# pymc-devs/nutpie

Hardware: AMD Instinct MI355X
Metric: leapfrog steps/sec (all chains) (higher is better)
Workload: dtype f64

## Files before the change

### nutpie_amd/csrc/kernels.hip

```cpp
#include <hip/hip_runtime.h>

#include "../../include/nphip_spec.h"
#include "engine_types.h"
#include "kernel_families.h"

#if defined(__HIP_DEVICE_COMPILE__)
#define NPHIP_GLOBAL __attribute__((address_space(1)))
#define NPHIP_LDS __attribute__((address_space(3)))
#define NPHIP_CONST __attribute__((address_space(4)))
#else
#define NPHIP_GLOBAL
#define NPHIP_LDS
#define NPHIP_CONST
#endif

#ifdef NPHIP_JIT_DENSITY
#define NPHIP_JIT 1
#else
#define NPHIP_JIT 0
#endif

namespace nphip {


// ... 392 lines not shown
                                       LdsDouble edge_ = nullptr)
        : A(a), c(ctl), red(r), par(par_), ring(ring_), edge(edge_), chain(ch), gchain((uint32_t)(a.chain_offset + ch)) {
        lane = threadIdx.x & 63;
        wave = (W == 1) ? 0 : __builtin_amdgcn_readfirstlane((int)(threadIdx.x >> 6));
        D = a.dim; ld = a.ld; nch = ld / NPHIP_CHUNK;
        qp = a.qpool + (size_t)ch * a.nqpool * 2 * ld;
        pp = a.pslots + (size_t)ch * a.npslots * ((NV == -1 || LR) ? (size_t)a.pvec : (size_t)2) * ld;
        sig2 = a.sig2 + (size_t)ch * ld;
        est = a.est + (size_t)ch * 8 * ld;
        T = a.s.num_tune + a.s.num_draws;
        if (DENS) {
            extern __shared__ __attribute__((aligned(16))) double s_dyn_dens[];
            const int slot = (W == 1) ? __builtin_amdgcn_readfirstlane((int)(threadIdx.x >> 6)) : 0;
            dens_lds = (LdsDouble)s_dyn_dens + (size_t)slot * a.dens_lds_doubles;
            dens_shared = (LdsDouble)s_dyn_dens + (size_t)(W == 1 ? 4 : 1) * a.dens_lds_doubles;
            dens_rows = dens_shared + a.dens_shared_doubles + (size_t)slot * 2 * ld;
        }
    }

    __device__ __forceinline__ void qe_st(int64_t i, double2 v) const { st2_dense(A.qeval + (size_t)chain * D, i, D, v); }
    __device__ __forceinline__ double2 ge_ld(int64_t i) const {
        const double* row = A.geval + (size_t)chain * D;
        if (DG && !(A.dg_variant & 128)) {
            double2 v;
            v.x = (i < D) ? __hip_atomic_load(row + i, __ATOMIC_RELAXED, __HIP_MEMORY_SCOPE_AGENT) : 0.0;
            v.y = (i + 1 < D) ? __hip_atomic_load(row + i + 1, __ATOMIC_RELAXED, __HIP_MEMORY_SCOPE_AGENT) : 0.0;
            return v;
        }
        return ld2_dense(row, i, D);
    }
    __device__ __forceinline__ double* Q(int64_t b) const { return qp + (size_t)b * 2 * ld; }
    __device__ __forceinline__ double* G(int64_t b) const { return qp + (size_t)b * 2 * ld + ld; }
    __device__ __forceinline__ size_t pvec() const { return LRK ? (size_t)A.pvec : (size_t)2; }
    __device__ __forceinline__ double* P(int64_t s) const { return pp + (size_t)s * pvec() * ld; }
    __device__ __forceinline__ double* R(int64_t s) const { return pp + (size_t)s * pvec() * ld + ld; }
    __device__ __forceinline__ double* VEL(int64_t s) const { return pp + (size_t)s * pvec() * ld + 2 * ld; }
    static constexpr bool LRK = NV == -1 || LR;
    __device__ __forceinline__ bool lr_job() const { return LRK && A.lr_on != 0; }
    __device__ __forceinline__ const float* LRV(int j) const { return A.lr_V + ((size_t)chain * kLrMax + j) * ld; }
    __device__ __forceinline__ double* EST(int64_t e, int k) const { return est + (size_t)(e * 4 + k) * ld; }
    __device__ __forceinline__ bool leader() const { return lane == 0 && wave == 0; }
    template <int N>
    __device__ __forceinline__ void rsum(double (&v)[N]) {
        static_assert(N <= 16, "a reduction area holds 16 values per wave");
        reduceN<W, N, false, !LEAN>(v, red + (W > 1 ? rflip * 16 * W : 0));
        rflip ^= 1;
    }
    __device__ __forceinline__ void rsum2(double& a, double& b) {
        double v[2] = {a, b};
        rsum(v);
        a = v[0]; b = v[1];
    }
    __device__ __forceinline__ double2 sg2(int64_t i) const {
        if (sig_lds) { const double2 v = *(const NPHIP_LDS double2*)(sig_lds + i); return v; }
        return ld2(sig2, i);
    }
    __device__ __forceinline__ double sg1(int64_t i) const { return sig_lds ? sig_lds[i] : ld1(sig2, i); }

#define NPHIP_FOR_CHUNKS(i) for (int64_t cc_ = wave, i = cc_ * NPHIP_CHUNK + 2 * lane; cc_ < nch; cc_ += W, i = cc_ * NPHIP_CHUNK + 2 * lane)
    template <int U, class LoadT, class BodyT>
    __device__ __forceinline__ void chunks_pf(LoadT load, BodyT body) const {
        for (int64_t c0 = wave; c0 < nch; c0 += (int64_t)W * U) {
            decltype(load((int64_t)0)) v[U];
#pragma unroll
            for (int u = 0; u < U; ++u) {
                int64_t cc = c0 + (int64_t)u * W;
                cc = cc < nch ? cc : nch - 1;
                v[u] = load(cc * NPHIP_CHUNK + 2 * lane);
            }
#pragma unroll
            for (int u = 0; u < U; ++u) {
                const int64_t cc = c0 + (int64_t)u * W;
                if (cc < nch) body(cc * NPHIP_CHUNK + 2 * lane, v[u]);
            }
        }
    }
    static constexpr bool BATCHED = (W == 1);
#ifdef NPHIP_NO_PFRARE
    static constexpr bool PFRARE = false;
#else
    static constexpr bool PFRARE = FUSED && W == 1 && NV >= 2 && !LEAN;
#endif
    static constexpr bool ENDOUT = FUSED && W == 1 && NV >= 2 && !LEAN;
    template <class LoadT, class BodyT>
    __device__ __forceinline__ void chunks(LoadT load, BodyT body) const {
        if (nch > 2) chunks_pf<4>(load, body);
        else chunks_pf<2>(load, body);
    }
    struct V4 { double2 a, b, c, d; };

    __device__ void da_init(double step) {
        c->da_log_step = nphip_log(step);
        c->da_log_step_adapted = c->da_log_step;
        c->da_hbar = 0.0;
        c->da_mu = A.s.adapt_adam ? 0.0 : nphip_log(10.0 * step);
        c->adam_b1t = 1.0; c->adam_b2t = 1.0;
        c->da_count = 1;
    }
    __device__ void da_advance(double accept) {
        if (A.s.adapt_adam) {
            const double g = accept - A.s.target_accept;
            c->da_hbar = 0.9 * c->da_hbar + (1.0 - 0.9) * g;
            c->da_mu = 0.999 * c->da_mu + (1.0 - 0.999) * (g * g);
            c->adam_b1t = c->adam_b1t * 0.9; c->adam_b2t = c->adam_b2t * 0.999;
            const double mhat = c->da_hbar / (1.0 - c->adam_b1t), vhat = c->da_mu / (1.0 - c->adam_b2t);
            c->da_log_step = c->da_log_step + A.s.adam_lr * mhat / (sqrt(vhat) + 1e-8);
            c->da_log_step_adapted = c->da_log_step;
            c->da_count += 1;
            return;
        }
        const double cnt = (double)c->da_count;
        double w = 1.0 / (cnt + A.s.da_t0);
        c->da_hbar = (1.0 - w) * c->da_hbar + w * (A.s.target_accept - accept);
        c->da_log_step = c->da_mu - c->da_hbar * sqrt(cnt) / A.s.da_gamma;
        double mk = nphip_exp(-A.s.da_k * nphip_log(cnt));
        c->da_log_step_adapted = mk * c->da_log_step + (1.0 - mk) * c->da_log_step_adapted;
        c->da_count += 1;
    }
    __device__ void update_stepsize(int64_t draw, bool best) {
        if (A.s.fixed_step_size) return;
        double step = best ? nphip_exp(c->da_log_step_adapted) : nphip_exp(c->da_log_step);
        if (A.s.jitter > 0.0) {
            nphip_u32x4 r = nphip_philox(A.s.seed, 0u, gchain, (uint32_t)draw, NPHIP_RNG_JITTER);
            double u = nphip_u01(r.v[0], r.v[1]);
            step *= fma(2.0 * A.s.jitter, u, 1.0 - A.s.jitter);
        }
        if (step > A.s.max_step_size) step = A.s.max_step_size;
        c->step_size = step;
    }
    __device__ int64_t alloc_q(bool in_tree) const {
        uint32_t used = 1u << c->cand_q;
        if (in_tree) {
            used |= (1u << c->endq[0]) | (1u << c->endq[1]) | (1u << c->curq);
            for (uint64_t m = (uint64_t)c->nleaf & ((1ull << kMaxDepthCap) - 1); m != 0; m &= m - 1) used |= 1u << c->sub_q[__builtin_ctzll(m)];
        }
        return (int64_t)__builtin_ctz(~used);
    }
    __device__ void finish_chain(int64_t phase, int64_t err) {
        c->phase = phase;
        c->err = err;
        if (leader()) atomicAdd(&A.counters[phase == PH_ERROR ? 1 : 0], 1ull);
    }

    __device__ void gen_init(int64_t attempt) {
        double* q = Q(0);
        NPHIP_FOR_CHUNKS(i) {
            double2 v = {0.0, 0.0};
            if (A.s.init_kind == 2) {
                v = ld2_dense(A.init_points + (size_t)chain * D, i, D);
            } else if (i < D) {
                nphip_u32x4 r = nphip_philox(A.s.seed, (uint32_t)(i >> 1), gchain, (uint32_t)attempt, NPHIP_RNG_INIT);
                if (A.s.init_kind == 0) {
                    v.x = fma(4.0, nphip_u01(r.v[0], r.v[1]), -2.0);
                    v.y = fma(4.0, nphip_u01(r.v[2], r.v[3]), -2.0);
                } else {
                    nphip_normal_pair(r, &v.x, &v.y);
                }
                if (i + 1 >= D) v.y = 0.0;
            }
            st2(q, i, v);
            if (!FUSED) qe_st(i, v);
        }
        c->eval_buf = 0;
    }

    struct LrAcc { double2 a[kLrMax]; };
// ... 1136 lines not shown
    __device__ __forceinline__ void regs_grad(RegsT& X) {
        double2 z[NVX];
#pragma unroll
        for (int k = 0; k < NVX; ++k) {
            const double2 mu = par_mu(ridx(k));
            z[k].x = X.q[k].x - mu.x;
            z[k].y = X.q[k].y - mu.y;
        }
        publish_edges(z);
#pragma unroll
        for (int k = 0; k < NVX; ++k) {
            double2 a, b01;
            double b2, edge_zl, edge_zr;
            par_ab(ridx(k), a, b01, b2);
            edge_pair(z, k, edge_zl, edge_zr);
            const double zl = wave_shr1(z[k].y, edge_zl), zr = wave_shl1(z[k].x, edge_zr);
            double tx = a.x * z[k].x;
            tx = fma(b01.x, zl, tx);
            tx = fma(b01.y, z[k].y, tx);
            double ty = a.y * z[k].y;
            ty = fma(b01.y, z[k].x, ty);
            ty = fma(b2, zr, ty);
            X.g[k].x = -tx;
            X.g[k].y = -ty;
        }
        if (W > 1) __syncthreads();
    }
    __device__ __forceinline__ void store_state(RegsT& X, bool q_, bool pr) {
        constexpr int nk = NVX;
        if (q_) {
            double* qn = Q(X.reg_q);
#pragma unroll
            for (int k = 0; k < NVX; ++k) if (k < nk) st2(qn, ridx(k), X.q[k]);
            if (REMOTE) {
                double* gn = G(X.reg_q);
#pragma unroll
                for (int k = 0; k < NVX; ++k) if (k < nk) st2(gn, ridx(k), X.g[k]);
            }
            X.dirty_qg = false;
        }
        if (pr) {
            double *pn = P(X.reg_p), *rn = R(X.reg_p);
#pragma unroll
            for (int k = 0; k < NVX; ++k) if (k < nk) { st2(pn, ridx(k), X.p[k]); st2(rn, ridx(k), X.r[k]); }
            if (LR) {
                double* vn = VEL(X.reg_p);
#pragma unroll
                for (int k = 0; k < NVX; ++k) st2(vn, ridx(k), X.v[k]);
            }
            X.dirty_pr = false;
        }
    }
    __device__ __forceinline__ void flush(RegsT& X) {
        if (NV <= 0) return;
        if (X.dirty_qg || X.dirty_pr) { if (LEAN) lean_store(lean_rs(), X, X.dirty_qg, X.dirty_pr); else store_state(X, X.dirty_qg, X.dirty_pr); }
        if (c->phase == PH_TREE) {
            if (LEAN) {
                lean_ring_flush(lean_rs(), X);
            } else {
                const int64_t d = c->depth;
                if (X.ring_leaf0 >= 0) flush_ring_slot(0, first_slot_of(X.ring_leaf0, d));
                if (X.ring_leaf1 >= 0) flush_ring_slot(1, slot_last(__builtin_ctzll((unsigned long long)X.ring_leaf1), A.cap));
            }
        }
    }
    __device__ __forceinline__ void flush_ring_slot(int sl, int64_t slot) {
        constexpr int nk = NVX;
        double2 tp[NVX], tr[NVX];
        ring_read(sl, tp, tr);
        double *pn = P(slot), *rn = R(slot);
#pragma unroll
        for (int k = 0; k < NVX; ++k) if (k < nk) { st2(pn, ridx(k), tp[k]); st2(rn, ridx(k), tr[k]); }
    }

    struct Hot {
        int32_t nleaf, depth, dir, idx_cur;
        int32_t srcq, srcp, newq, newp;
        int32_t n_steps, n_steps0;
        int32_t end_newp;
        uint32_t used_base, sub_used, draw;
        bool check;
        double step, H0, acc, acc_sym, max_ee;
    };
    static __device__ __forceinline__ int32_t end_code(bool diverging, bool maxdepth, bool store_div, bool div_has_end, bool regrad, bool replay) {
        return 1 | (diverging ? 2 : 0) | (maxdepth ? 4 : 0) | (store_div ? 8 : 0) | (div_has_end ? 16 : 0) | (regrad ? 32 : 0) | (replay ? 64 : 0);
    }
    static __device__ __forceinline__ int32_t rfl(int64_t v) { return __builtin_amdgcn_readfirstlane((int)v); }
    static __device__ __forceinline__ double rfl_f64(double v) {
        return __hiloint2double(__builtin_amdgcn_readfirstlane(__double2hiint(v)), __builtin_amdgcn_readfirstlane(__double2loint(v)));
    }
    __device__ __forceinline__ void hot_doubling(Hot& H) const {
        const int db = H.dir > 0 ? 1 : 0;
        H.used_base = (1u << rfl(c->cand_q)) | (1u << rfl(c->endq[0])) | (1u << rfl(c->endq[1]));
        H.end_newp = slot_end(db, (int)(rfl(c->endpar[db]) ^ 1));
        H.check = A.s.check_turning && ((int64_t)H.depth + 1 > A.s.mindepth);
    }
    __device__ __forceinline__ void hot_load(Hot& H) const {
        H.nleaf = rfl(c->nleaf); H.depth = rfl(c->depth); H.dir = rfl(c->dir); H.idx_cur = rfl(c->idx_cur);
        H.srcq = rfl(c->lf_srcq); H.srcp = rfl(c->lf_srcp); H.newq = rfl(c->lf_newq); H.newp = rfl(c->lf_newp);
        H.n_steps = H.n_steps0 = rfl(c->n_steps); H.draw = (uint32_t)rfl(c->draw);
        H.step = rfl_f64(c->step_size); H.H0 = rfl_f64(c->H0); H.acc = rfl_f64(c->acc_sum); H.acc_sym = rfl_f64(c->acc_sym_sum);
        H.max_ee = A.s.max_energy_error;
        hot_doubling(H);
        H.sub_used = 0u;
        for (uint32_t m = (uint32_t)H.nleaf & ((1u << kMaxDepthCap) - 1u); m != 0; m &= m - 1) H.sub_used |= 1u << rfl(c->sub_q[__builtin_ctz(m)]);
    }
    __device__ __forceinline__ void hot_save(Hot& H) {
        c->nleaf = H.nleaf; c->dir = H.dir; c->idx_cur = H.idx_cur;
        c->lf_srcq = H.srcq; c->lf_srcp = H.srcp; c->lf_newq = H.newq; c->lf_newp = H.newp; c->lf_sign = H.dir; c->eval_buf = H.newq;
        c->curq = H.srcq; c->curp = H.srcp;
        c->n_steps = H.n_steps; c->total_steps += (int64_t)(H.n_steps - H.n_steps0);
        H.n_steps0 = H.n_steps;
        c->acc_sum = H.acc; c->acc_sym_sum = H.acc_sym;
    }
    __device__ __forceinline__ void issue_leaf_hot(Hot& H) const {
        const int32_t j = H.nleaf + 1, d = H.depth;
        int32_t newp;
        if (j == (1 << d)) newp = H.end_newp;
        else if (j & 1) newp = (j == 1) ? slot_first(d) : slot_first(__builtin_ctz((unsigned)(j - 1)));
        else newp = slot_last(__builtin_ctz((unsigned)j), A.cap);
        H.newq = (int32_t)__builtin_ctz(~(H.used_base | H.sub_used | (1u << H.srcq)));
        H.newp = newp;
    }
    __device__ __forceinline__ void start_doubling_hot(Hot& H) const {
        nphip_u32x4 r = nphip_philox(A.s.seed, (uint32_t)H.depth, gchain, H.draw, NPHIP_RNG_DIRECTION);
        H.dir = (r.v[0] & 1u) ? 1 : -1;
        const int db = H.dir > 0 ? 1 : 0;
        H.nleaf = 0;
        H.srcq = rfl(c->endq[db]);
        H.srcp = rfl(c->endp[db]);
        H.idx_cur = rfl(H.dir > 0 ? c->idx_right : c->idx_left);
        H.sub_used = 0u;
        hot_doubling(H);
        issue_leaf_hot(H);
    }
    __device__ __forceinline__ double merge_uniform_hot(const Hot& H, int32_t j, int32_t d, int32_t k, nphip_u32x4& blk, int32_t& blk_id) const {
        const int32_t id = k >> 1;
        if (blk_id != id) {
            const uint32_t c3 = (uint32_t)NPHIP_RNG_MERGE | ((uint32_t)d << 8) | ((uint32_t)id << 16);
            blk = nphip_philox(A.s.seed, (uint32_t)j, gchain, H.draw, c3);
            blk_id = id;
        }
        return (k & 1) ? nphip_u01(blk.v[2], blk.v[3]) : nphip_u01(blk.v[0], blk.v[1]);
    }

    __device__ __forceinline__ void merge_level(Hot& H, int32_t j, int32_t d, int32_t k, nphip_u32x4& blk, int32_t& blk_id, double& T_wm, int64_t& T_we,
                                                int32_t& T_q, double& T_U, double& T_E, int32_t& T_idx) {
        double sm; int64_t se;
        const int32_t A_q = rfl(c->sub_q[k]), A_idx = rfl(c->sub_idx[k]);
        const double A_U = c->sub_U[k], A_E = c->sub_E[k];
        H.sub_used &= ~(1u << A_q);
        nphip_w_add(c->sub_wm[k], c->sub_we[k], T_wm, T_we, &sm, &se);
        const bool take = merge_uniform_hot(H, j, d, k, blk, blk_id) * sm < nphip_w_rel(T_wm, T_we, se);
        if (!take) { T_q = A_q; T_U = A_U; T_E = A_E; T_idx = A_idx; }
        T_wm = sm; T_we = se;
    }

    __device__ __forceinline__ bool leaf_reg(RegsT& X, Hot& H, int32_t& end_code_out) {
        constexpr int nk = NVX;
        const int32_t j = H.nleaf + 1, d = H.depth, dir = H.dir;
        const int db = dir > 0 ? 1 : 0;
        const int32_t idx_new = H.idx_cur + dir;
        const int32_t srcq = H.srcq, srcp = H.srcp, newq = H.newq, newp = H.newp;
        const bool check = H.check;
#ifdef NPHIP_PROFILE
        const int64_t tp0 = (int64_t)__builtin_readcyclecounter();
#endif
        if (X.reg_q != srcq) {
            const double* q = Q(srcq);
#pragma unroll
            for (int k = 0; k < NVX; ++k) if (k < nk) X.q[k] = ld2(q, ridx(k));
            if (REMOTE) {
                const double* g = G(srcq);
#pragma unroll
                for (int k = 0; k < NVX; ++k) if (k < nk) X.g[k] = ld2(g, ridx(k));
            } else {
                regs_grad(X);
            }
        }
        if (X.reg_p != srcp) { load_slot(srcp, X.p, X.r); if (LR) load_slot_v(srcp, X.v); }
        if (!X.sig_ok) {
#pragma unroll
            for (int k = 0; k < NVX; ++k) if (k < nk) X.s[k] = ld2(sig2, ridx(k));
            if (LR) {
                const double* sdp = A.lr_std + (size_t)chain * ld;
#pragma unroll
                for (int k = 0; k < NVX; ++k) X.sd[k] = ld2(sdp, ridx(k));
            }
            X.sig_ok = true;
        }
        if (j == 1) { X.ring_leaf0 = -1; X.ring_leaf1 = -1; }
        const bool lrm = LR && lr_job() && rfl(c->host_metric) != 0;
        const int lrk = lrm ? (int)rfl(c->lr_k) : 0;
        NPHIP_PHASE_FENCE();
        const double eps = (double)dir * H.step;
        const double h = 0.5 * eps;
        if (idx_new == -1) {
#pragma unroll
            for (int k = 0; k < NVX; ++k) if (k < nk) { X.r[k].x = -0.0; X.r[k].y = -0.0; }
        }
        double2 z[NVX], pold[NVX], rold[NVX], vold[NVX];
        LrAcc lrS;
        double lrc[kLrMax];
        if (LR && lrm) lr_zero(lrS);
#pragma unroll
        for (int k = 0; k < NVX; ++k) if (k < nk) {
            pold[k] = X.p[k];
            rold[k] = X.r[k];
            if (LR) vold[k] = X.v[k];
            X.p[k].x = fma(h, X.g[k].x, X.p[k].x);
            X.p[k].y = fma(h, X.g[k].y, X.p[k].y);
            if (LR && lrm) {
            } else {
                X.q[k].x = fma(eps, X.s[k].x * X.p[k].x, X.q[k].x);
                X.q[k].y = fma(eps, X.s[k].y * X.p[k].y, X.q[k].y);
            }
            if (!REMOTE && !(LR && lrm)) {
                const double2 mu = par_mu(ridx(k));
                z[k].x = X.q[k].x - mu.x;
                z[k].y = X.q[k].y - mu.y;
            }
        }
        if (LR && lrm) {
            lr_dispatch(lrk, [&](auto kc) {
#pragma unroll
                for (int k = 0; k < NVX; ++k) {
                    double2 u;
                    u.x = X.sd[k].x * X.p[k].x; u.y = X.sd[k].y * X.p[k].y;
                    lr_acc_c<decltype(kc)::value>(lrS, ridx(k), u);
                }
            });
            lr_coef(lrS, lrk, 0, lrc);
            lr_dispatch(lrk, [&](auto kc) {
#pragma unroll
                for (int k = 0; k < NVX; ++k) {
                    double2 u;
                    u.x = X.sd[k].x * X.p[k].x; u.y = X.sd[k].y * X.p[k].y;
                    const double2 w = lr_apply_c<decltype(kc)::value>(ridx(k), u, lrc);
                    X.q[k].x = fma(eps, X.sd[k].x * w.x, X.q[k].x);
                    X.q[k].y = fma(eps, X.sd[k].y * w.y, X.q[k].y);
                }
            });
            if (!REMOTE) {
#pragma unroll
                for (int k = 0; k < NVX; ++k) {
                    const double2 mu = par_mu(ridx(k));
                    z[k].x = X.q[k].x - mu.x;
                    z[k].y = X.q[k].y - mu.y;
                }
            }
        }
        double lp_remote = 0.0;
        int64_t code_remote = 0;
        if (REMOTE) {
            if (DENS) {
#pragma unroll
                for (int k = 0; k < NVX; ++k) if (k < nk) *(NPHIP_LDS double2*)(dens_rows + ridx(k)) = X.q[k];
                remote_eval(lp_remote, code_remote, true);
            } else {
#pragma unroll
                for (int k = 0; k < NVX; ++k) if (k < nk) qe_st(ridx(k), X.q[k]);
                remote_eval(lp_remote, code_remote, false, !DG);
            }
        } else {
            publish_edges(z);
        }
        double2 accK = {0.0, 0.0}, accL = {0.0, 0.0}, accE = {0.0, 0.0}, accS = {0.0, 0.0};
        if (LR && lrm) lr_zero(lrS);
#pragma unroll
        for (int k = 0; k < NVX; ++k) if (k < nk) {
            double2 gg;
            if (DENS) {
                gg = *(const NPHIP_LDS double2*)(dens_rows + ld + ridx(k));
                if (ridx(k) >= D) gg.x = 0.0;
                if (ridx(k) + 1 >= D) gg.y = 0.0;
            } else if (REMOTE) {
                gg = ge_ld(ridx(k));
                if (DG) {
                    const double2 mu = ld2(A.dg_mu, ridx(k));
                    accL.x = fma(X.q[k].x - mu.x, gg.x, accL.x);
                    accL.y = fma(X.q[k].y - mu.y, gg.y, accL.y);
                }
            } else {
                double2 a, b01;
                double b2, edge_zl, edge_zr;
                par_ab(ridx(k), a, b01, b2);
                edge_pair(z, k, edge_zl, edge_zr);
                const double zl = wave_shr1(z[k].y, edge_zl);
                const double zr = wave_shl1(z[k].x, edge_zr);
                double tx = a.x * z[k].x;
                tx = fma(b01.x, zl, tx);
                tx = fma(b01.y, z[k].y, tx);
                double ty = a.y * z[k].y;
                ty = fma(b01.y, z[k].x, ty);
                ty = fma(b2, zr, ty);
                gg.x = -tx;
                gg.y = -ty;
                accL.x = fma(z[k].x, gg.x, accL.x);
                accL.y = fma(z[k].y, gg.y, accL.y);
            }
            X.g[k] = gg;
            X.p[k].x = fma(h, gg.x, X.p[k].x);
            X.p[k].y = fma(h, gg.y, X.p[k].y);
            X.r[k].x = rold[k].x + X.p[k].x;
            X.r[k].y = rold[k].y + X.p[k].y;
            if (LR && lrm) continue;
            const double vx = X.s[k].x * X.p[k].x, vy = X.s[k].y * X.p[k].y;
            accK.x = fma(X.p[k].x, vx, accK.x);
            accK.y = fma(X.p[k].y, vy, accK.y);
            const double tx0 = (X.r[k].x - rold[k].x) + pold[k].x, ty0 = (X.r[k].y - rold[k].y) + pold[k].y;
            accE.x = fma(tx0, vx, accE.x);
            accE.y = fma(ty0, vy, accE.y);
            if (LR) {
                X.v[k].x = vx; X.v[k].y = vy;
                accS.x = fma(tx0, vold[k].x, accS.x);
                accS.y = fma(ty0, vold[k].y, accS.y);
            } else {
                accS.x = fma(tx0, X.s[k].x * pold[k].x, accS.x);
                accS.y = fma(ty0, X.s[k].y * pold[k].y, accS.y);
            }
        }
        if (LR && lrm) {
            lr_dispatch(lrk, [&](auto kc) {
#pragma unroll
                for (int k = 0; k < NVX; ++k) {
                    double2 u;
                    u.x = X.sd[k].x * X.p[k].x; u.y = X.sd[k].y * X.p[k].y;
                    lr_acc_c<decltype(kc)::value>(lrS, ridx(k), u);
                }
            });
            lr_coef(lrS, lrk, 0, lrc);
            lr_dispatch(lrk, [&](auto kc) {
#pragma unroll
                for (int k = 0; k < NVX; ++k) {
                    double2 u;
                    u.x = X.sd[k].x * X.p[k].x; u.y = X.sd[k].y * X.p[k].y;
                    const double2 w = lr_apply_c<decltype(kc)::value>(ridx(k), u, lrc);
                    X.v[k].x = X.sd[k].x * w.x; X.v[k].y = X.sd[k].y * w.y;
                }
            });
#pragma unroll
            for (int k = 0; k < NVX; ++k) {
                accK.x = fma(X.p[k].x, X.v[k].x, accK.x);
                accK.y = fma(X.p[k].y, X.v[k].y, accK.y);
                const double tx0 = (X.r[k].x - rold[k].x) + pold[k].x, ty0 = (X.r[k].y - rold[k].y) + pold[k].y;
                accE.x = fma(tx0, X.v[k].x, accE.x);
                accE.y = fma(ty0, X.v[k].y, accE.y);
                accS.x = fma(tx0, vold[k].x, accS.x);
                accS.y = fma(ty0, vold[k].y, accS.y);
            }
        }
        X.reg_q = newq;
        X.reg_p = newp;
        X.dirty_qg = true;
        X.dirty_pr = true;
        if (!LR && !NORING) {
            if ((j & 3) == 1) { ring_write(0, X.p, X.r); X.ring_leaf0 = j; }
            else if ((j & 3) == 2) { ring_write(1, X.p, X.r); X.ring_leaf1 = j; }
        }
#ifdef NPHIP_PROFILE
        const int64_t tp1 = (int64_t)__builtin_readcyclecounter();
#endif
        NPHIP_PHASE_FENCE();
        double v4[4] = {accK.x + accK.y, accL.x + accL.y, accE.x + accE.y, accS.x + accS.y};
        rsum(v4);
        NPHIP_PHASE_FENCE();
#ifdef NPHIP_PROFILE
        const int64_t tp2 = (int64_t)__builtin_readcyclecounter();
        c->prof[0] += tp1 - tp0; c->prof[6] += tp2 - tp1;
#endif
        const double K = 0.5 * v4[0], lp = (REMOTE && !DG) ? lp_remote : 0.5 * v4[1];
        const bool turn0 = (v4[2] < 0.0) || (v4[3] < 0.0);
        if (REMOTE && code_remote < 0) { X.dirty_qg = X.dirty_pr = false; hot_save(H); finish_chain(PH_ERROR, CE_FATAL_LOGP); return true; }
        H.nleaf += 1;
        H.n_steps += 1;
        const bool ok = isfinite(lp) && (!REMOTE || code_remote == 0);
        const double Unew = -lp, E = K + Unew, dE = E - H.H0;
        const bool diverged = !ok || (dE > H.max_ee) || !isfinite(dE);
        double T_wm = 1.0;
        int64_t T_we = 0;
        nphip_u32x4 mrg_blk = {{0u, 0u, 0u, 0u}};
        int32_t mrg_id = -1;
        {
            if (!diverged) {
                const double x = -dE, xc = x > 1e9 ? 1e9 : (x < -1e9 ? -1e9 : x);
                double kk;
                nphip_exp_parts(xc, &T_wm, &kk);
                T_we = (int64_t)kk;
                const double e = nphip_exp_scale(x, T_wm, kk);
                const double a = e < 1.0 ? e : 1.0;
                H.acc += a;
                H.acc_sym += 2.0 * a / (1.0 + e);
            }
        }
        if (diverged) { X.dirty_qg = X.dirty_pr = false; hot_save(H);
            if (ENDOUT) end_code_out = end_code(true, false, FUSED, ok, !REMOTE, FUSED); else rare_end_draw(A, c, red, chain, true, false, FUSED, ok, !REMOTE, FUSED);
            return true; }
#ifdef NPHIP_PROFILE
        int64_t tq = (int64_t)__builtin_readcyclecounter();
        c->prof[8] += tq - tp2;
#endif

        NPHIP_PHASE_FENCE();
        double T_U = Unew, T_E = E;
        int32_t T_q = newq, T_idx = idx_new;
        H.srcq = newq; H.srcp = newp; H.idx_cur = idx_new;
        double2 obp[NVX], obr[NVX], obv[NVX];
        int32_t k = 0;
        while (k < d && (((j - 1) >> k) & 1)) {
            if (check) {
                bool turn;
                if (k == 0) {
                    turn = turn0;
                } else if (LR) {
                    const int32_t a = j - (2 << k) + 1, al = j - (1 << k);
                    load_slot(first_slot_of(a, d), obp, obr); load_slot_v(first_slot_of(a, d), obv);
                    if (k == 2) { load_slot(first_slot_of(al + 1, d), pold, rold); load_slot_v(first_slot_of(al + 1, d), vold); }
                    turn = sub_a_v(X, obp, obr, obv, pold, rold, vold);
                    if (k >= 2) {
#pragma unroll
                        for (int q_ = 0; q_ < NVX; ++q_) { pold[q_] = obp[q_]; rold[q_] = obr[q_]; vold[q_] = obv[q_]; }
                    }
                    if (!turn) {
                        const int32_t sl_ = slot_last(__builtin_ctz((unsigned)al), A.cap);
                        load_slot(sl_, obp, obr); load_slot_v(sl_, obv);
                        turn = sub_b_v(X, obp, obr, obv);
                    }
                } else {
                    const int32_t a = j - (2 << k) + 1, al = j - (1 << k);
                    if (k == 1 && X.ring_leaf0 == a) ring_read(0, obp, obr);
                    else load_slot(first_slot_of(a, d), obp, obr);
                    if (k == 2) {
                        if (X.ring_leaf0 == al + 1) ring_read(0, pold, rold);
                        else load_slot(first_slot_of(al + 1, d), pold, rold);
                    }
                    turn = sub_a(X, obp, obr, pold, rold);
                    if (k >= 2) {
#pragma unroll
                        for (int q_ = 0; q_ < NVX; ++q_) { pold[q_] = obp[q_]; rold[q_] = obr[q_]; }
                    }
                    if (!turn) {
                        if (k == 1 && X.ring_leaf1 == al) ring_read(1, obp, obr);
                        else load_slot(slot_last(__builtin_ctz((unsigned)al), A.cap), obp, obr);
                        turn = sub_b(X, obp, obr);
                    }
                }
                if (turn) { X.dirty_qg = X.dirty_pr = false; hot_save(H); if (ENDOUT) end_code_out = end_code(false, false, false, false, !REMOTE, false); else rare_end_draw(A, c, red, chain, false, false, false, false, !REMOTE); return true; }
            }
#ifdef NPHIP_PROFILE
            { const int64_t t_ = (int64_t)__builtin_readcyclecounter(); c->prof[k == 0 ? 9 : 10] += t_ - tq; tq = t_; }
#endif
            NPHIP_PHASE_FENCE();
            merge_level(H, j, d, k, mrg_blk, mrg_id, T_wm, T_we, T_q, T_U, T_E, T_idx);
            NPHIP_PHASE_FENCE();
#ifdef NPHIP_PROFILE
            { const int64_t t_ = (int64_t)__builtin_readcyclecounter(); c->prof[11] += t_ - tq; tq = t_; }
#endif
            ++k;
        }
        if (k < d) {
            c->sub_wm[k] = T_wm; c->sub_we[k] = T_we; c->sub_q[k] = T_q; c->sub_U[k] = T_U; c->sub_E[k] = T_E; c->sub_idx[k] = T_idx;
            H.sub_used |= 1u << T_q;
#ifdef NPHIP_PROFILE
            const int64_t tp3 = (int64_t)__builtin_readcyclecounter();
#endif
            store_state(X, T_q == newq, LR || NORING || ((j & 3) == 0) || ((j & 7) == 1));
            issue_leaf_hot(H);
#ifdef NPHIP_PROFILE
            c->prof[7] += (int64_t)__builtin_readcyclecounter() - tp3;
#endif
            return false;
        }
        bool turn = false;
        if (check) {
            const int32_t far_slot = rfl(c->endp[1 - db]), far_idx = rfl(dir > 0 ? c->idx_left : c->idx_right);
            const int32_t near_idx = rfl(dir > 0 ? c->idx_right : c->idx_left);
            if (d == 0) {
                turn = LR ? check1_v(X, pold, pold, vold, far_idx, idx_new) : check1(X, pold, pold, far_idx, idx_new);
            } else if (LR) {
                if (d == 2) { load_slot(slot_first((int)d), pold, rold); load_slot_v(slot_first((int)d), vold); }
                load_slot(far_slot, obp, obr); load_slot_v(far_slot, obv);
                turn = check_a_v(X, obp, obr, obv, pold, rold, vold, far_idx, near_idx + dir, idx_new);
                if (!turn) {
                    load_slot(rfl(c->endp[db]), obp, obr); load_slot_v(rfl(c->endp[db]), obv);
                    turn = check1_v(X, obp, obr, obv, near_idx, idx_new);
                }
            } else {
                if (d == 2) {
                    if (X.ring_leaf0 == 1) ring_read(0, pold, rold);
                    else load_slot(slot_first((int)d), pold, rold);
                }
                load_slot(far_slot, obp, obr);
                turn = check_a(X, obp, obr, pold, rold, far_idx, near_idx + dir, idx_new);
                if (!turn) {
                    load_slot(rfl(c->endp[db]), obp, obr);
                    turn = check1(X, obp, obr, near_idx, idx_new);
                }
            }
        }
        c->endq[db] = newq;
        c->endp[db] = newp;
        c->endpar[db] ^= 1;
        if (dir > 0) c->idx_right = idx_new; else c->idx_left = idx_new;
        {
            double sm; int64_t se;
            nphip_w_add(c->main_wm, c->main_we, T_wm, T_we, &sm, &se);
            const double ref = nphip_w_rel(c->main_wm, c->main_we, se), oth = nphip_w_rel(T_wm, T_we, se);
            bool take = oth >= ref;
            if (!take) take = merge_uniform_hot(H, j, d, d, mrg_blk, mrg_id) * ref < oth;
            if (take) { c->cand_q = T_q; c->cand_U = T_U; c->cand_E = T_E; c->cand_idx = T_idx; }
            c->main_wm = sm; c->main_we = se;
            H.depth = d + 1;
            c->depth = d + 1;
        }
        store_state(X, true, true);
        if (turn) { hot_save(H); if (ENDOUT) end_code_out = end_code(false, false, false, false, !REMOTE, false); else rare_end_draw(A, c, red, chain, false, false, false, false, !REMOTE); return true; }
        if (H.depth >= A.s.maxdepth) { hot_save(H); if (ENDOUT) end_code_out = end_code(false, true, false, false, !REMOTE, false); else rare_end_draw(A, c, red, chain, false, true, false, false, !REMOTE); return true; }
        start_doubling_hot(H);
        return false;
    }

    typedef unsigned int u32x4 __attribute__((ext_vector_type(4)));
    typedef unsigned int u32x2 __attribute__((ext_vector_type(2)));
    struct LeanRs {
        __amdgpu_buffer_rsrc_t q, p, mu, a, b;
        uint32_t voff;
        uint32_t wave_off;
    };
    static __device__ __forceinline__ __amdgpu_buffer_rsrc_t mk_rsrc(const void* ptr, uint64_t bytes) {
        const uint64_t v = (uint64_t)ptr;
        const uint32_t lo = (uint32_t)__builtin_amdgcn_readfirstlane((int)(uint32_t)v), hi = (uint32_t)__builtin_amdgcn_readfirstlane((int)(uint32_t)(v >> 32));
        return __builtin_amdgcn_make_buffer_rsrc((void*)(((uint64_t)hi << 32) | lo), 0, (int)__builtin_amdgcn_readfirstlane((int)(uint32_t)bytes), 0x00020000);
    }
    __device__ __forceinline__ LeanRs lean_rs() const {
        LeanRs r;
        r.q = mk_rsrc(qp, (uint64_t)A.nqpool * 2 * ld * 8);
        r.p = mk_rsrc(pp, (uint64_t)A.npslots * 2 * ld * 8);
        r.mu = mk_rsrc(A.m_mu, (uint64_t)ld * 8);
        r.a = mk_rsrc(A.m_a, (uint64_t)ld * 8);
        r.b = mk_rsrc(A.m_bsh, (uint64_t)(ld + 8) * 8);
        r.voff = (uint32_t)lane * 16u;
        r.wave_off = (uint32_t)wave * (NPHIP_CHUNK * 8);
        return r;
    }
    __device__ __forceinline__ uint32_t soff(const LeanRs& rs, int64_t slot, int vec, int k) const {
        const uint32_t s_ = (uint32_t)__builtin_amdgcn_readfirstlane((int)slot);
        return (s_ * 2u + (uint32_t)vec) * (uint32_t)(ld * 8) + (uint32_t)k * (uint32_t)(W * NPHIP_CHUNK * 8) + rs.wave_off;
    }
    static __device__ __forceinline__ double2 bld2(__amdgpu_buffer_rsrc_t r, uint32_t voff, uint32_t so) {
        return __builtin_bit_cast(double2, __builtin_amdgcn_raw_buffer_load_b128(r, (int)voff, (int)so, 0));
    }
    static __device__ __forceinline__ void bst2(__amdgpu_buffer_rsrc_t r, uint32_t voff, uint32_t so, double2 v) {
        __builtin_amdgcn_raw_buffer_store_b128(__builtin_bit_cast(u32x4, v), r, (int)voff, (int)so, 0);
    }
    __device__ __forceinline__ double2 par2(const LeanRs& rs, __amdgpu_buffer_rsrc_t r, int k) const {
        return bld2(r, rs.voff, (uint32_t)k * (uint32_t)(W * NPHIP_CHUNK * 8) + rs.wave_off);
    }
    __device__ __forceinline__ double par_b2(const LeanRs& rs, int k) const {
        return __builtin_bit_cast(double, __builtin_amdgcn_raw_buffer_load_b64(rs.b, (int)(rs.voff + 16u), (int)((uint32_t)k * (uint32_t)(W * NPHIP_CHUNK * 8) + rs.wave_off), 0));
    }
    __device__ __forceinline__ double2 sigl(const LeanRs& rs, int k) const {
        return *(const NPHIP_LDS double2*)((const NPHIP_LDS char*)sig_lds + ((uint32_t)k * (uint32_t)(W * NPHIP_CHUNK * 8) + rs.wave_off + rs.voff));
    }

    static constexpr int LR_FREE = LEAN ? lean_free_chunks(W, NVX) : 0;
    static constexpr int KP = LR_FREE < 0 ? 0 : (LR_FREE < NVX ? LR_FREE : NVX);
    static constexpr int KR = (LR_FREE - KP) < 0 ? 0 : ((LR_FREE - KP) < NVX ? (LR_FREE - KP) : NVX);
    static constexpr bool LRING = KP > 0;
    __device__ __forceinline__ NPHIP_LDS double2* lring(const LeanRs& rs, int vec, int k) const {
        return (NPHIP_LDS double2*)((NPHIP_LDS char*)sig_lds + (uint32_t)(ld * 8) + (uint32_t)((vec == 0 ? 0 : KP) + k) * (uint32_t)(W * NPHIP_CHUNK * 8) +
                                    rs.wave_off + rs.voff);
    }
    __device__ __forceinline__ void lean_ring_flush(const LeanRs& rs, RegsT& X) {
        if (!LRING || X.ring_leaf1 < 0) return;
        const int64_t slot = slot_last(__builtin_ctzll((unsigned long long)X.ring_leaf1), A.cap);
#pragma unroll
        for (int k = 0; k < NVX; ++k) {
            if (k < KP) bst2(rs.p, rs.voff, soff(rs, slot, 0, k), *lring(rs, 0, k));
            if (k < KR) bst2(rs.p, rs.voff, soff(rs, slot, 1, k), *lring(rs, 1, k));
        }
        X.ring_leaf1 = -1;
    }

    __device__ __forceinline__ void lean_grad(const LeanRs& rs, RegsT& X) {
#pragma unroll
        for (int k = 0; k < NVX; ++k) {
            const double2 mu = par2(rs, rs.mu, k);
            const int64_t cch = (int64_t)k * W + wave;
            const double zx = X.q[k].x - mu.x, zy = X.q[k].y - mu.y;
            if (lane == 0 || lane == 63) edge[2 * cch + (lane == 0 ? 1 : 2)] = (lane == 0) ? zx : zy;
            NPHIP_CHUNK_FENCE(k);
        }
        __syncthreads();
#pragma unroll
        for (int k = 0; k < NVX; ++k) {
            const int64_t cch = (int64_t)k * W + wave;
            const double2 mu = par2(rs, rs.mu, k), a = par2(rs, rs.a, k), b01 = par2(rs, rs.b, k);
            const double b2 = par_b2(rs, k);
            double2 z;
            z.x = X.q[k].x - mu.x;
            z.y = X.q[k].y - mu.y;
// ... 1020 lines not shown
        const float* sv = A.st_V + (size_t)chain * kLrMax * ld;
        float* lv = A.lr_V + (size_t)chain * kLrMax * ld;
        NPHIP_FOR_CHUNKS(i) {
            const double2 v = ld2(s2, i);
            st2(sig2, i, v);
            double2 r; r.x = sqrt(v.x); r.y = sqrt(v.y);
            st2(sd, i, r);
            for (int j = 0; j < kLrMax; ++j) *(NPHIP_GLOBAL float2*)(lv + (size_t)j * ld + i) = *(const NPHIP_GLOBAL float2*)(sv + (size_t)j * ld + i);
        }
        if (wave == 0 && lane < kLrMax) A.lr_lam[(size_t)chain * kLrMax + lane] = A.st_lam[(size_t)chain * kLrMax + lane];
        __builtin_amdgcn_fence(__ATOMIC_SEQ_CST, "workgroup");
        __builtin_amdgcn_s_dcache_inv();
        if (W > 1) __syncthreads();
        c->host_metric = 1;
        c->lr_k = k;
        c->staged = 0;
    }

    __device__ __forceinline__ void rare_phase(int64_t ph) {
        double lp = 0.0;
        int64_t code = 0;
        if (ph == PH_START) {
            c->init_attempt = 0;
            gen_init(0);
            c->phase = PH_INIT_EVAL;
            if (FUSED) chain_sync<W>();
        } else if (ph == PH_RESUME_SS) {
            c->has_initial_mm = 0;
            start_ss(0x80000000ll | c->draw);
        } else if (ph == PH_DRAW_BEGIN) {
            begin_draw(true);
        } else if (ph == PH_INIT_EVAL) {
            eval_position(c->eval_buf, lp, code);
            cont_init(lp, code);
            if (FUSED && c->phase == PH_INIT_EVAL) chain_sync<W>();
        } else {
            double K = lf2(lp, code, c->lf_sign);
            if (code < 0) { finish_chain(PH_ERROR, CE_FATAL_LOGP); return; }
            cont_ss(K, lp, code, ph == PH_SS_FIRST);
        }
    }

    __device__ __forceinline__ void run(int budget, bool have, LdsDouble sig_copy = nullptr, bool materialise = false) {
        if (!INK && materialise && c->phase == PH_TREE) {
            lf1(c->lf_srcq, c->lf_srcp, c->lf_newq, c->lf_newp, c->lf_sign);
        }
        bool worked = false;
        for (;;) {
            const int64_t ph = c->phase;
            if (ph == PH_DONE || ph == PH_ERROR || ph == PH_WAIT_HOST) {
                if (REMOTE && !DENS && !DG) { while (c->hs_last == 0) remote_sync(); }
                break;
            }
            if (SLICED && (ph == PH_DRAW_END || ph == PH_DRAW_BEGIN)) {
                if (worked) break;
                if (ph == PH_DRAW_END) {
                    const int64_t pe = c->pend_end;
                    rare_end_draw(A, c, red, chain, (pe & 1) != 0, (pe & 2) != 0, (pe & 4) != 0, (pe & 8) != 0, NOG);
                } else {
                    rare_phase_fn(A, c, red, chain, ph);
                }
                break;
            }
            if (ph != PH_START && ph != PH_RESUME_SS) {
                if (REMOTE && !DENS && !DG) {
                    if (c->hs_last != 0) break;
                } else if (FUSED || DENS || DG) {
                    if (budget <= 0) break;
                    --budget;
                } else {
                    if (!have) break;
                    have = false;
                }
            }
            worked = true;
            if (ph != PH_TREE) {
                rare_phase_fn(A, c, red, chain, ph);
                continue;
            }
            RegsT X;
            SCacheT Y;
            Hot H;
            constexpr bool HOT = NV > 0;
            if (HOT) hot_load(H);
            int32_t end_code_ = 0;
            bool rare = false, out_of_budget = false;
            int lean_end = 0;
            const LeanRs lrs = lean_rs();
            if ((NV == 0 || NV == -1 || LEAN) && sig_copy != nullptr) {
                for (int64_t i = 2 * (int64_t)threadIdx.x; i < ld; i += 2 * (int64_t)blockDim.x)
                    *(NPHIP_LDS double2*)(sig_copy + i) = ld2(sig2, i);
                __syncthreads();
                sig_lds = sig_copy;
            }
            for (;;) {
#ifdef NPHIP_PROFILE
                const int64_t t0 = (int64_t)__builtin_readcyclecounter();
#endif
                if (NV > 0) {
                    if (LEAN) { lean_end = leaf_lean(lrs, X, H); rare = lean_end != 0; }
                    else rare = leaf_reg(X, H, end_code_);
                } else {
                    double lp = 0.0;
                    int64_t code = 0;
                    if (FUSED && !lr_job()) {
                        bool turn0 = false;
                        const bool even_leaf = ((c->nleaf + 1) & 1) == 0;
                        const double K = lf_stream(lp, c->idx_cur + c->dir, turn0, Y);
                        rare = cont_tree(X, Y, K, lp, code, even_leaf, turn0);
                    } else {
                        if (FUSED) lf1(c->lf_srcq, c->lf_srcp, c->lf_newq, c->lf_newp, c->lf_sign);
                        CbCrit cr;
                        bool fast = false;
                        if (cb_fast_ok()) {
                            lp = A.ueval[chain];
                            code = A.ecode ? A.ecode[chain] : 0;
                            fast = code == 0 && isfinite(lp);
                        }
                        const double K = fast ? leaf_cb(cr) : lf2(lp, code, c->idx_cur + c->dir);
#ifdef NPHIP_PROFILE
                        c->prof[0] += (int64_t)__builtin_readcyclecounter() - t0;
#endif
                        rare = cont_tree(X, Y, K, lp, code, false, false, fast ? &cr : nullptr);
                    }
                }
#ifdef NPHIP_PROFILE
                const int64_t t2 = (int64_t)__builtin_readcyclecounter();
                c->prof[3] += 1;
                if (rare) { c->prof[2] += t2 - t0; c->prof[5] += 1; } else { c->prof[1] += t2 - t0; c->prof[4] += 1; }
#endif
                if (rare || (!HOT && c->phase != PH_TREE)) break;
                if (REMOTE && !DENS && !DG) {
                    if (c->hs_last != 0) { out_of_budget = true; break; }
                } else if (FUSED || DENS || DG) {
                    if (budget <= 0) { out_of_budget = true; break; }
                    --budget;
                } else {
                    out_of_budget = true;
                    break;
                }
            }
            if (!rare) {
                if (HOT) hot_save(H);
                flush(X);
            }
            sig_lds = nullptr;
            if (ENDOUT && end_code_ != 0) {
                const int32_t ec = end_code_;
                rare_end_draw(A, c, red, chain, (ec & 2) != 0, (ec & 4) != 0, (ec & 8) != 0, (ec & 16) != 0, (ec & 32) != 0, (ec & 64) != 0);
            }
            if (LEAN && lean_end != 0) rare_end_draw(A, c, red, chain, lean_end == 1 || lean_end == 4, lean_end == 3, lean_end == 1 || lean_end == 4, lean_end == 1, true, true);
            if (out_of_budget) break;
        }
    }
#undef NPHIP_FOR_CHUNKS
};

template <bool FUSED, int W, int NV, bool LEAN = false, bool REMOTE = false, bool LR = false, bool WIDE = false, bool DENSEG = false>
__global__ __launch_bounds__(W == 1 ? 256 : 64 * W) __attribute__((amdgpu_waves_per_eu(min_waves<FUSED, W, NV, LEAN, REMOTE, LR, WIDE>(), max_waves<FUSED, W, NV, LEAN, REMOTE, LR, WIDE>())))
void k_advance(const Args* __restrict__ Ap, int max_evals, int have_result, const LaunchSlice sl) {
    const NPHIP_CONST Args& A = *(const NPHIP_CONST Args*)Ap;
    constexpr int WAVES = (W == 1) ? 4 : W;
    __shared__ Ctl s_ctl[WAVES];
    __shared__ double s_red[W == 1 ? 8 : 32 * WAVES];
    __shared__ __attribute__((aligned(16))) double s_par[(NV > 0 && W == 1) ? 3 * 128 * NV + 8 : 2];
    __shared__ __attribute__((aligned(16))) double s_ring[(NV > 0 && !LEAN && !LR && !(W == 1 && NV > 8)) ? WAVES * 4 * 128 * NV : 2];
    __shared__ double s_edge[(NV > 0 && W > 1) ? 2 * W * NV + 2 : 2];
    extern __shared__ __attribute__((aligned(16))) double s_dyn[];
    const int wib = __builtin_amdgcn_readfirstlane((int)(threadIdx.x >> 6)), lane = threadIdx.x & 63;
    const int cpb = (W == 1 && REMOTE && NPHIP_JIT != 0) ? sl.cpb : 4;
    const int64_t chain = sl.chain_lo + ((W == 1) ? (int64_t)blockIdx.x * cpb + wib : (int64_t)blockIdx.x);
    if (NV > 0 && W == 1 && !REMOTE) {
        const int64_t ld = A.ld;
        NPHIP_LDS double* sp = (NPHIP_LDS double*)s_par;
        for (int64_t i = threadIdx.x; i < ld; i += blockDim.x) {
            sp[i] = ld1(A.m_mu, i);
            sp[ld + i] = ld1(A.m_a, i);
            sp[2 * ld + i] = (i == 0) ? -0.0 : ld1(A.m_b, i - 1);
        }
        if (threadIdx.x < 8) sp[3 * ld + threadIdx.x] = -0.0;
        __syncthreads();
    }
#if NPHIP_JIT
    if (REMOTE) {
// ... 569 lines not shown
```

Baseline: 245.9 million.

## Hoist sampler args into scalar registers and retire vector loads early in leaf

Adds a HotArgs struct that caches seed, maxdepth, turning-check threshold and cap in scalar registers once per tree. The leaf step, merge and doubling helpers now read these instead of reloading kernel arguments on each leaf. It also inserts explicit vmcnt(0) waits after state loads so later code does not carry partial waits, and adds an optional (off by default) two-ahead prefetch of the density parameters. This trades extra SGPR pressure and earlier stalls for fewer redundant argument loads.

```diff
diff --git a/nutpie_amd/csrc/kernels.hip b/nutpie_amd/csrc/kernels.hip
--- a/nutpie_amd/csrc/kernels.hip
+++ b/nutpie_amd/csrc/kernels.hip
@@ -498,6 +498,22 @@
     static constexpr bool PFRARE = FUSED && W == 1 && NV >= 2 && !LEAN;
 #endif
     static constexpr bool ENDOUT = FUSED && W == 1 && NV >= 2 && !LEAN;
+    static constexpr bool LEAFWAITS = FUSED && NV > 0 && !LEAN && !LR && !(W == 1 && NV == 3 && TAG == 0) && !(W == 4 && NV == 2);
+#ifdef NPHIP_NO_VMRETIRE
+    static constexpr bool VMRETIRE = false;
+#else
+    static constexpr bool VMRETIRE = LEAFWAITS;
+#endif
+#ifdef NPHIP_PARAHEAD
+    static constexpr int PARAHEAD = (FUSED && W == 1 && NV >= 3 && !LEAN && !LR) ? NPHIP_PARAHEAD : 0;
+#else
+    static constexpr int PARAHEAD = 0;
+#endif
+#ifdef NPHIP_NO_HOTARGS
+    static constexpr bool HOTARGS = false;
+#else
+    static constexpr bool HOTARGS = LEAFWAITS;
+#endif
     template <class LoadT, class BodyT>
     __device__ __forceinline__ void chunks(LoadT load, BodyT body) const {
         if (nch > 2) chunks_pf<4>(load, body);
@@ -1800,6 +1816,23 @@
         bool check;
         double step, H0, acc, acc_sym, max_ee;
     };
+    struct HotArgs {
+        uint64_t seed;
+        int32_t maxdepth;
+        int32_t check_from;
+        int32_t cap;
+    };
+    static __device__ __forceinline__ void keep_s(int32_t& v) { asm volatile("" : "+s"(v)); }
+    static __device__ __forceinline__ void keep_s(uint64_t& v) {
+        int32_t lo = (int32_t)(uint32_t)v, hi = (int32_t)(uint32_t)(v >> 32);
+        keep_s(lo); keep_s(hi);
+        v = ((uint64_t)(uint32_t)hi << 32) | (uint64_t)(uint32_t)lo;
+    }
+    static __device__ __forceinline__ void keep_s(double& v) {
+        int32_t lo = __double2loint(v), hi = __double2hiint(v);
+        keep_s(lo); keep_s(hi);
+        v = __hiloint2double(hi, lo);
+    }
     static __device__ __forceinline__ int32_t end_code(bool diverging, bool maxdepth, bool store_div, bool div_has_end, bool regrad, bool replay) {
         return 1 | (diverging ? 2 : 0) | (maxdepth ? 4 : 0) | (store_div ? 8 : 0) | (div_has_end ? 16 : 0) | (regrad ? 32 : 0) | (replay ? 64 : 0);
     }
@@ -1862,6 +1895,49 @@
         return (k & 1) ? nphip_u01(blk.v[2], blk.v[3]) : nphip_u01(blk.v[0], blk.v[1]);
     }
 
+    __device__ __forceinline__ void hot_args_load(Hot& H, HotArgs& HA) const {
+        const int64_t mind = A.s.mindepth;
+        HA.seed = A.s.seed; HA.maxdepth = (int32_t)A.s.maxdepth; HA.cap = A.cap;
+        HA.check_from = !A.s.check_turning ? 2 * kMaxDepthCap : (mind < 0 ? -1 : (mind > 2 * kMaxDepthCap ? 2 * kMaxDepthCap : (int32_t)mind));
+        keep_s(H.max_ee); keep_s(HA.seed); keep_s(HA.maxdepth); keep_s(HA.check_from); keep_s(HA.cap);
+    }
+    __device__ __forceinline__ void hot_doubling(Hot& H, const HotArgs& HA) const {
+        const int db = H.dir > 0 ? 1 : 0;
+        H.used_base = (1u << rfl(c->cand_q)) | (1u << rfl(c->endq[0])) | (1u << rfl(c->endq[1]));
+        H.end_newp = slot_end(db, (int)(rfl(c->endpar[db]) ^ 1));
+        H.check = H.depth + 1 > HA.check_from;
+    }
+    __device__ __forceinline__ void issue_leaf_hot(Hot& H, const HotArgs& HA) const {
+        const int32_t j = H.nleaf + 1, d = H.depth;
+        int32_t newp;
+        if (j == (1 << d)) newp = H.end_newp;
+        else if (j & 1) newp = (j == 1) ? slot_first(d) : slot_first(__builtin_ctz((unsigned)(j - 1)));
+        else newp = slot_last(__builtin_ctz((unsigned)j), HA.cap);
+        H.newq = (int32_t)__builtin_ctz(~(H.used_base | H.sub_used | (1u << H.srcq)));
+        H.newp = newp;
+    }
+    __device__ __forceinline__ void start_doubling_hot(Hot& H, const HotArgs& HA) const {
+        nphip_u32x4 r = nphip_philox(HA.seed, (uint32_t)H.depth, gchain, H.draw, NPHIP_RNG_DIRECTION);
+        H.dir = (r.v[0] & 1u) ? 1 : -1;
+        const int db = H.dir > 0 ? 1 : 0;
+        H.nleaf = 0;
+        H.srcq = rfl(c->endq[db]);
+        H.srcp = rfl(c->endp[db]);
+        H.idx_cur = rfl(H.dir > 0 ? c->idx_right : c->idx_left);
+        H.sub_used = 0u;
+        hot_doubling(H, HA);
+        issue_leaf_hot(H, HA);
+    }
+    __device__ __forceinline__ double merge_uniform_hot(const Hot& H, const HotArgs& HA, int32_t j, int32_t d, int32_t k, nphip_u32x4& blk, int32_t& blk_id) const {
+        const int32_t id = k >> 1;
+        if (blk_id != id) {
+            const uint32_t c3 = (uint32_t)NPHIP_RNG_MERGE | ((uint32_t)d << 8) | ((uint32_t)id << 16);
+            blk = nphip_philox(HA.seed, (uint32_t)j, gchain, H.draw, c3);
+            blk_id = id;
+        }
+        return (k & 1) ? nphip_u01(blk.v[2], blk.v[3]) : nphip_u01(blk.v[0], blk.v[1]);
+    }
+
     __device__ __forceinline__ void merge_level(Hot& H, int32_t j, int32_t d, int32_t k, nphip_u32x4& blk, int32_t& blk_id, double& T_wm, int64_t& T_we,
                                                 int32_t& T_q, double& T_U, double& T_E, int32_t& T_idx) {
         double sm; int64_t se;
@@ -1874,7 +1950,19 @@
         T_wm = sm; T_we = se;
     }
 
-    __device__ __forceinline__ bool leaf_reg(RegsT& X, Hot& H, int32_t& end_code_out) {
+    __device__ __forceinline__ void merge_level(Hot& H, const HotArgs& HA, int32_t j, int32_t d, int32_t k, nphip_u32x4& blk, int32_t& blk_id, double& T_wm, int64_t& T_we,
+                                                int32_t& T_q, double& T_U, double& T_E, int32_t& T_idx) {
+        double sm; int64_t se;
+        const int32_t A_q = rfl(c->sub_q[k]), A_idx = rfl(c->sub_idx[k]);
+        const double A_U = c->sub_U[k], A_E = c->sub_E[k];
+        H.sub_used &= ~(1u << A_q);
+        nphip_w_add(c->sub_wm[k], c->sub_we[k], T_wm, T_we, &sm, &se);
+        const bool take = merge_uniform_hot(H, HA, j, d, k, blk, blk_id) * sm < nphip_w_rel(T_wm, T_we, se);
+        if (!take) { T_q = A_q; T_U = A_U; T_E = A_E; T_idx = A_idx; }
+        T_wm = sm; T_we = se;
+    }
+
+    __device__ __forceinline__ bool leaf_reg(RegsT& X, Hot& H, const HotArgs HA, int32_t& end_code_out) {
         constexpr int nk = NVX;
         const int32_t j = H.nleaf + 1, d = H.depth, dir = H.dir;
         const int db = dir > 0 ? 1 : 0;
@@ -1895,8 +1983,9 @@
             } else {
                 regs_grad(X);
             }
-        }
-        if (X.reg_p != srcp) { load_slot(srcp, X.p, X.r); if (LR) load_slot_v(srcp, X.v); }
+            if (VMRETIRE) wait_vm0();
+        }
+        if (X.reg_p != srcp) { load_slot(srcp, X.p, X.r); if (LR) load_slot_v(srcp, X.v); if (VMRETIRE) wait_vm0(); }
         if (!X.sig_ok) {
 #pragma unroll
             for (int k = 0; k < NVX; ++k) if (k < nk) X.s[k] = ld2(sig2, ridx(k));
@@ -1906,6 +1995,7 @@
                 for (int k = 0; k < NVX; ++k) X.sd[k] = ld2(sdp, ridx(k));
             }
             X.sig_ok = true;
+            if (VMRETIRE) wait_vm0();
         }
         if (j == 1) { X.ring_leaf0 = -1; X.ring_leaf1 = -1; }
         const bool lrm = LR && lr_job() && rfl(c->host_metric) != 0;
@@ -1921,8 +2011,12 @@
         LrAcc lrS;
         double lrc[kLrMax];
         if (LR && lrm) lr_zero(lrS);
+        double2 mu_pf[NVX], a_pf[NVX], b01_pf[NVX];
+        double b2_pf[NVX];
+        if (PARAHEAD) { mu_pf[0] = par_mu(ridx(0)); mu_pf[1] = par_mu(ridx(1)); }
 #pragma unroll
         for (int k = 0; k < NVX; ++k) if (k < nk) {
+            if (PARAHEAD && k + 2 < NVX) mu_pf[k + 2 < NVX ? k + 2 : 0] = par_mu(ridx(k + 2));
             pold[k] = X.p[k];
             rold[k] = X.r[k];
             if (LR) vold[k] = X.v[k];
@@ -1934,10 +2028,11 @@
                 X.q[k].y = fma(eps, X.s[k].y * X.p[k].y, X.q[k].y);
             }
             if (!REMOTE && !(LR && lrm)) {
-                const double2 mu = par_mu(ridx(k));
+                const double2 mu = PARAHEAD ? mu_pf[k] : par_mu(ridx(k));
                 z[k].x = X.q[k].x - mu.x;
                 z[k].y = X.q[k].y - mu.y;
             }
+            if (PARAHEAD == 1) NPHIP_CHUNK_FENCE(k);
         }
         if (LR && lrm) {
             lr_dispatch(lrk, [&](auto kc) {
@@ -1985,8 +2080,10 @@
         }
         double2 accK = {0.0, 0.0}, accL = {0.0, 0.0}, accE = {0.0, 0.0}, accS = {0.0, 0.0};
         if (LR && lrm) lr_zero(lrS);
+        if (PARAHEAD) { par_ab(ridx(0), a_pf[0], b01_pf[0], b2_pf[0]); par_ab(ridx(1), a_pf[1], b01_pf[1], b2_pf[1]); }
 #pragma unroll
         for (int k = 0; k < NVX; ++k) if (k < nk) {
+            if (PARAHEAD && k + 2 < NVX) { const int kk = k + 2 < NVX ? k + 2 : 0; par_ab(ridx(k + 2), a_pf[kk], b01_pf[kk], b2_pf[kk]); }
             double2 gg;
             if (DENS) {
                 gg = *(const NPHIP_LDS double2*)(dens_rows + ld + ridx(k));
@@ -2002,7 +2099,7 @@
             } else {
                 double2 a, b01;
                 double b2, edge_zl, edge_zr;
-                par_ab(ridx(k), a, b01, b2);
+                if (PARAHEAD) { a = a_pf[k]; b01 = b01_pf[k]; b2 = b2_pf[k]; } else par_ab(ridx(k), a, b01, b2);
                 edge_pair(z, k, edge_zl, edge_zr);
                 const double zl = wave_shr1(z[k].y, edge_zl);
                 const double zr = wave_shl1(z[k].x, edge_zr);
@@ -2037,6 +2134,7 @@
                 accS.x = fma(tx0, X.s[k].x * pold[k].x, accS.x);
                 accS.y = fma(ty0, X.s[k].y * pold[k].y, accS.y);
             }
+            if (PARAHEAD == 1) NPHIP_CHUNK_FENCE(k);
         }
         if (LR && lrm) {
             lr_dispatch(lrk, [&](auto kc) {
@@ -2140,7 +2238,7 @@
                         for (int q_ = 0; q_ < NVX; ++q_) { pold[q_] = obp[q_]; rold[q_] = obr[q_]; vold[q_] = obv[q_]; }
                     }
                     if (!turn) {
-                        const int32_t sl_ = slot_last(__builtin_ctz((unsigned)al), A.cap);
+                        const int32_t sl_ = slot_last(__builtin_ctz((unsigned)al), HOTARGS ? HA.cap : A.cap);
                         load_slot(sl_, obp, obr); load_slot_v(sl_, obv);
                         turn = sub_b_v(X, obp, obr, obv);
                     }
@@ -2159,7 +2257,7 @@
                     }
                     if (!turn) {
                         if (k == 1 && X.ring_leaf1 == al) ring_read(1, obp, obr);
-                        else load_slot(slot_last(__builtin_ctz((unsigned)al), A.cap), obp, obr);
+                        else load_slot(slot_last(__builtin_ctz((unsigned)al), HOTARGS ? HA.cap : A.cap), obp, obr);
                         turn = sub_b(X, obp, obr);
                     }
                 }
@@ -2169,7 +2267,8 @@
             { const int64_t t_ = (int64_t)__builtin_readcyclecounter(); c->prof[k == 0 ? 9 : 10] += t_ - tq; tq = t_; }
 #endif
             NPHIP_PHASE_FENCE();
-            merge_level(H, j, d, k, mrg_blk, mrg_id, T_wm, T_we, T_q, T_U, T_E, T_idx);
+            if (HOTARGS) merge_level(H, HA, j, d, k, mrg_blk, mrg_id, T_wm, T_we, T_q, T_U, T_E, T_idx);
+            else merge_level(H, j, d, k, mrg_blk, mrg_id, T_wm, T_we, T_q, T_U, T_E, T_idx);
             NPHIP_PHASE_FENCE();
 #ifdef NPHIP_PROFILE
             { const int64_t t_ = (int64_t)__builtin_readcyclecounter(); c->prof[11] += t_ - tq; tq = t_; }
@@ -2183,7 +2282,7 @@
             const int64_t tp3 = (int64_t)__builtin_readcyclecounter();
 #endif
             store_state(X, T_q == newq, LR || NORING || ((j & 3) == 0) || ((j & 7) == 1));
-            issue_leaf_hot(H);
+            if (HOTARGS) issue_leaf_hot(H, HA); else issue_leaf_hot(H);
 #ifdef NPHIP_PROFILE
             c->prof[7] += (int64_t)__builtin_readcyclecounter() - tp3;
 #endif
@@ -2225,7 +2324,7 @@
             nphip_w_add(c->main_wm, c->main_we, T_wm, T_we, &sm, &se);
             const double ref = nphip_w_rel(c->main_wm, c->main_we, se), oth = nphip_w_rel(T_wm, T_we, se);
             bool take = oth >= ref;
-            if (!take) take = merge_uniform_hot(H, j, d, d, mrg_blk, mrg_id) * ref < oth;
+            if (!take) take = (HOTARGS ? merge_uniform_hot(H, HA, j, d, d, mrg_blk, mrg_id) : merge_uniform_hot(H, j, d, d, mrg_blk, mrg_id)) * ref < oth;
             if (take) { c->cand_q = T_q; c->cand_U = T_U; c->cand_E = T_E; c->cand_idx = T_idx; }
             c->main_wm = sm; c->main_we = se;
             H.depth = d + 1;
@@ -2233,8 +2332,8 @@
         }
         store_state(X, true, true);
         if (turn) { hot_save(H); if (ENDOUT) end_code_out = end_code(false, false, false, false, !REMOTE, false); else rare_end_draw(A, c, red, chain, false, false, false, false, !REMOTE); return true; }
-        if (H.depth >= A.s.maxdepth) { hot_save(H); if (ENDOUT) end_code_out = end_code(false, true, false, false, !REMOTE, false); else rare_end_draw(A, c, red, chain, false, true, false, false, !REMOTE); return true; }
-        start_doubling_hot(H);
+        if (HOTARGS ? H.depth >= HA.maxdepth : H.depth >= A.s.maxdepth) { hot_save(H); if (ENDOUT) end_code_out = end_code(false, true, false, false, !REMOTE, false); else rare_end_draw(A, c, red, chain, false, true, false, false, !REMOTE); return true; }
+        if (HOTARGS) start_doubling_hot(H, HA); else start_doubling_hot(H);
         return false;
     }
 
@@ -3421,7 +3520,9 @@
             SCacheT Y;
             Hot H;
             constexpr bool HOT = NV > 0;
+            HotArgs HA;
             if (HOT) hot_load(H);
+            if (HOTARGS) hot_args_load(H, HA);
             int32_t end_code_ = 0;
             bool rare = false, out_of_budget = false;
             int lean_end = 0;
@@ -3438,7 +3539,7 @@
 #endif
                 if (NV > 0) {
                     if (LEAN) { lean_end = leaf_lean(lrs, X, H); rare = lean_end != 0; }
-                    else rare = leaf_reg(X, H, end_code_);
+                    else rare = leaf_reg(X, H, HA, end_code_);
                 } else {
                     double lp = 0.0;
                     int64_t code = 0;
```

After: 244.1 million. About the same (-0.8%).
